# youmi-zym/GO-SLAM

Measured on AMD Instinct MI355X. Metric: BA keyframes/s (6 x FactorGraph.update: reproject + corr lookup + GRU + 2 GN BA iters) on synthetic 640x480 RGB-D, higher is better.
Workload: dtype f32 (BA/geometry; fp64 solve), f16 (corr volume, GRU convs); 1 GPU; configs[1]-shaped frontend window: 60x80 maps (480x640 RGB-D), P=25 keyframes, E=75 edges, 6 updates/keyframe, iters=2, RGB-D depth prior, upsample on; parallelism=replicas x1 (tracking does not shard)

## Files before the change

go_slam_amd/csrc/ba.hip:

```cpp
#include "common.h"

int gs_chol_solve_launch(double* H, double* b, int n, float lm, float ep, float* dx_out, int32_t* fail_flag,
                         int32_t* fail_count, hipStream_t st);

namespace {

constexpr float kMinDepth = 0.25f;
constexpr float kAlpha = 0.05f;
constexpr int kPrepThreads = 1024;
constexpr int kAccSplit = 4;
constexpr int kMaxBuf = 4096;

struct BaWs {
  int32_t* hdr;
  int32_t* kinv;
  int32_t* kx;
  int32_t* edge_m;
  int32_t* row_ptr;
  int32_t* csr_edge;
  int32_t* ent_ptr;
  int32_t* ent_src;
  int32_t* ent_pose;
  int32_t* pair_ptr;
  float* Q;
  float* W;
  float* Ei;
  float* Eij;
  float* part;
  double* H;
  double* b;
  size_t total;
};

BaWs carve(void* base, int E, int P, int M, int nbuf, int hw) {
  BaWs w;
  size_t off = 0;
  auto take = [&](size_t bytes) { size_t o = off; off += gs_align(bytes); return (char*)base + o; };
  w.hdr = (int32_t*)take(16 * 4);
  w.kinv = (int32_t*)take((size_t)nbuf * 4);
  w.kx = (int32_t*)take((size_t)(M + 1) * 4);
  w.edge_m = (int32_t*)take((size_t)(E + 1) * 4);
  w.row_ptr = (int32_t*)take((size_t)(M + 2) * 4);
  w.csr_edge = (int32_t*)take((size_t)(E + 1) * 4);
  w.ent_ptr = (int32_t*)take((size_t)(M + 2) * 4);
  w.ent_src = (int32_t*)take((size_t)(M + E + 1) * 4);
  w.ent_pose = (int32_t*)take((size_t)(M + E + 1) * 4);
  w.pair_ptr = (int32_t*)take((size_t)(M + 2) * 4);
  w.Q = (float*)take((size_t)M * hw * 4);
  w.W = (float*)take((size_t)M * hw * 4);
  w.Ei = (float*)take((size_t)M * 6 * hw * 4);
  w.Eij = (float*)take((size_t)E * 6 * hw * 4);
  w.part = (float*)take((size_t)kAccSplit * M * 8 * hw * 4);
  const size_t n = (size_t)6 * P;
  w.H = (double*)take((n * n + n) * 8);
  w.b = w.H + n * n;
  w.total = off;
  return w;
}

__device__ void block_exclusive_scan(int* data, int n, int* scratch , int* total) {
  const int tid = threadIdx.x;
  const int per = (n + kPrepThreads - 1) / kPrepThreads;
  const int beg = min(tid * per, n), end = min(beg + per, n);
  int s = 0;
  for (int i = beg; i < end; ++i) s += data[i];
  scratch[tid] = s;
  __syncthreads();
  for (int off = 1; off < kPrepThreads; off <<= 1) {
    int v = (tid >= off) ? scratch[tid - off] : 0;
    __syncthreads();
    scratch[tid] += v;
    __syncthreads();
  }
  int run = scratch[tid] - s;
  for (int i = beg; i < end; ++i) {
    int v = data[i];
    data[i] = run;
    run += v;
  }
  if (tid == kPrepThreads - 1) *total = scratch[tid];
  __syncthreads();
}

__global__ __launch_bounds__(kPrepThreads) void ba_prep_kernel(
    const int64_t* __restrict__ ii, const int64_t* __restrict__ jj, int E, int nbuf, int t0, int t1,
    int M_host, BaWs w) {
  __shared__ int flag[kMaxBuf];
  __shared__ int cnt_a[kMaxBuf];
  __shared__ int cnt_b[kMaxBuf];
  __shared__ int scratch[kPrepThreads];
  __shared__ int total;
  const int tid = threadIdx.x;

  for (int k = tid; k < nbuf; k += kPrepThreads) flag[k] = (k >= t0 && k < t1) ? 1 : 0;
  __syncthreads();
  for (int e = tid; e < E; e += kPrepThreads) {
    const int i = (int)ii[e];
    if (i >= 0 && i < nbuf) flag[i] = 1;
  }
  __syncthreads();
  for (int k = tid; k < nbuf; k += kPrepThreads) cnt_a[k] = flag[k];
  __syncthreads();
  block_exclusive_scan(flag, nbuf, scratch, &total);
  const int M_dev = total;
  const int M = min(M_dev, M_host);
  for (int k = tid; k < nbuf; k += kPrepThreads) {
    const bool mem = cnt_a[k] != 0;
    const int r = flag[k];
    const int row = (mem && r < M) ? r : -1;
    w.kinv[k] = row;
    if (row >= 0) w.kx[row] = k;
  }
  if (tid == 0) {
    w.hdr[0] = M_dev;
    w.hdr[1] = (M_dev != M_host) ? 1 : 0;
    w.hdr[2] = 0;
    w.hdr[3] = 0;
  }
  __syncthreads();
  for (int m = tid; m < kMaxBuf; m += kPrepThreads) { cnt_a[m] = 0; cnt_b[m] = 0; }
  __syncthreads();
  for (int k = tid; k < nbuf; k += kPrepThreads) {
    const int row = w.kinv[k];
    if (row >= 0 && k >= t0 && k < t1) cnt_b[row] = 1;
  }
  __syncthreads();
  for (int e = tid; e < E; e += kPrepThreads) {
    const int i = (int)ii[e], j = (int)jj[e];
    const int row = (i >= 0 && i < nbuf) ? w.kinv[i] : -1;
    w.edge_m[e] = row;
    if (row >= 0) {
      atomicAdd(&cnt_a[row], 1);
      if (j >= t0 && j < t1) atomicAdd(&cnt_b[row], 1);
    }
  }
  __syncthreads();
  for (int m = tid; m < M_host; m += kPrepThreads) flag[m] = cnt_b[m] * cnt_b[m];
  __syncthreads();
  block_exclusive_scan(cnt_a, M_host, scratch, &total);
  if (tid == 0) w.row_ptr[M_host] = total;
  block_exclusive_scan(cnt_b, M_host, scratch, &total);
  if (tid == 0) w.ent_ptr[M_host] = total;
  block_exclusive_scan(flag, M_host, scratch, &total);
  if (tid == 0) { w.pair_ptr[M_host] = total; w.hdr[4] = total; }
  __syncthreads();
  for (int m = tid; m < M_host; m += kPrepThreads) {
    w.row_ptr[m] = cnt_a[m];
    w.ent_ptr[m] = cnt_b[m];
    w.pair_ptr[m] = flag[m];
  }
  __syncthreads();
  for (int m = tid; m < M; m += kPrepThreads) {
    int rp = cnt_a[m], ep = cnt_b[m];
    const int k = w.kx[m];
    if (k >= t0 && k < t1) { w.ent_src[ep] = m; w.ent_pose[ep] = k - t0; ++ep; }
    for (int e = 0; e < E; ++e) {
      if (w.edge_m[e] == m) {
        w.csr_edge[rp++] = e;
        const int j = (int)jj[e];
        if (j >= t0 && j < t1) { w.ent_src[ep] = M_host + e; w.ent_pose[ep] = j - t0; ++ep; }
      }
    }
  }
}
// ... 172 lines not shown
          if (j_in) gs_atomic_add_f64(&w.b[6 * pj_ + (tid - 84)], s);
        }
      }
      __syncthreads();
    }
  }

  if (!motion_only && active) {
    if (nsplit > 1) {
      float* po = w.part + (((size_t)split * gridDim.y + m) * 8) * hw + p;
      po[0] = Csum;
      po[(size_t)hw] = wsum;
#pragma unroll
      for (int n = 0; n < 6; ++n) po[(size_t)(2 + n) * hw] = Ei[n];
      return;
    }
    const size_t o = (size_t)m * hw + p;
    const float sens = disps_sens[(size_t)k * hw + p];
    const float mk = (sens > 0.0f) ? 1.0f : 0.0f;
    const float C = Csum + mk * kAlpha + (1.0f - mk) * eta[o];
    const float ww = wsum - mk * kAlpha * (disp - sens);
    w.Q[o] = 1.0f / C;
    w.W[o] = ww;
    if (i_in) {
      float* eo = w.Ei + ((size_t)m * 6) * hw + p;
#pragma unroll
      for (int n = 0; n < 6; ++n) eo[(size_t)n * hw] = Ei[n];
    }
  }
}

__global__ __launch_bounds__(256) void ba_accum_finish_kernel(const float* __restrict__ disps,
                                                              const float* __restrict__ disps_sens,
                                                              const float* __restrict__ eta, int t0, int t1, int hw, int nsp,
                                                              BaWs w) {
  const int m = blockIdx.y;
  if (m >= w.hdr[0]) return;
  const int nsplit = min(nsp, max(w.row_ptr[m + 1] - w.row_ptr[m], 1));
  if (nsplit <= 1) return;
  const int p = blockIdx.x * 256 + threadIdx.x;
  if (p >= hw) return;
  float acc[8];
#pragma unroll
  for (int n = 0; n < 8; ++n) acc[n] = 0.0f;
  for (int s2 = 0; s2 < nsplit; ++s2) {
    const float* pi_ = w.part + (((size_t)s2 * gridDim.y + m) * 8) * hw + p;
#pragma unroll
    for (int n = 0; n < 8; ++n) acc[n] += pi_[(size_t)n * hw];
  }
  const int k = w.kx[m];
  const size_t o = (size_t)m * hw + p;
  const float disp = disps[(size_t)k * hw + p];
  const float sens = disps_sens[(size_t)k * hw + p];
  const float mk = (sens > 0.0f) ? 1.0f : 0.0f;
  const float C = acc[0] + mk * kAlpha + (1.0f - mk) * eta[o];
  const float ww = acc[1] - mk * kAlpha * (disp - sens);
  w.Q[o] = 1.0f / C;
  w.W[o] = ww;
  const int pi = k - t0;
  if (pi >= 0 && pi < t1 - t0) {
    float* eo = w.Ei + ((size_t)m * 6) * hw + p;
#pragma unroll
    for (int n = 0; n < 6; ++n) eo[(size_t)n * hw] = acc[2 + n];
  }
}

__global__ __launch_bounds__(256) void ba_schur_kernel(int M, int hw, int P, BaWs w) {
  __shared__ float red[4][44];
  const int tid = threadIdx.x;
  const int wave = tid >> 6, lane = tid & 63;
  typedef const __attribute__((address_space(4))) int* cip;
  cip pair_ptr = (cip)w.pair_ptr, ent_ptr = (cip)w.ent_ptr, ent_pose = (cip)w.ent_pose, ent_src = (cip)w.ent_src;
  const int n_pairs = pair_ptr[M];
  const int n6 = 6 * P;
  for (int pidx = blockIdx.x; pidx < n_pairs; pidx += gridDim.x) {
    int lo = 0, hi = M;
    while (hi - lo > 1) {
      const int mid = (lo + hi) >> 1;
      if (pair_ptr[mid] <= pidx) lo = mid; else hi = mid;
    }
    const int m = lo;
    const int eb = ent_ptr[m];
    const int nm = ent_ptr[m + 1] - eb;
    const int r = pidx - pair_ptr[m];
    const int a = r / nm, b = r - a * nm;
    const int pa = ent_pose[eb + a], pb = ent_pose[eb + b];
    if (pa < pb) continue;
    const int sa = ent_src[eb + a], sb = ent_src[eb + b];
    const float* Ea = (sa < M) ? w.Ei + (size_t)sa * 6 * hw : w.Eij + (size_t)(sa - M) * 6 * hw;
    const float* Eb = (sb < M) ? w.Ei + (size_t)sb * 6 * hw : w.Eij + (size_t)(sb - M) * 6 * hw;
    const float* Qm = w.Q + (size_t)m * hw;
    const float* Wm = w.W + (size_t)m * hw;
    const bool diag = (a == b);
    float S[36];
#pragma unroll
    for (int i = 0; i < 36; ++i) S[i] = 0.f;
    float vv[6] = {0.f, 0.f, 0.f, 0.f, 0.f, 0.f};
    constexpr int UP = 4;
    for (int p0 = tid; p0 < hw; p0 += UP * 256) {
      float q[UP], ea[UP][6], eb_[UP][6], ww[UP];
#pragma unroll
      for (int u = 0; u < UP; ++u) {
        const int p = p0 + 256 * u;
        const bool ok = p < hw;
        const int pc = ok ? p : tid;
        q[u] = Qm[pc];
#pragma unroll
        for (int n = 0; n < 6; ++n) {
          ea[u][n] = Ea[(size_t)n * hw + pc];
          eb_[u][n] = Eb[(size_t)n * hw + pc];
        }
        ww[u] = diag ? Wm[pc] : 0.0f;
      }
#pragma unroll
      for (int u = 0; u < UP; ++u) {
        if (p0 + 256 * u < hw) {
#pragma unroll
          for (int n = 0; n < 6; ++n) ea[u][n] = ea[u][n] * q[u];
#pragma unroll
          for (int n = 0; n < 6; ++n)
#pragma unroll
            for (int c = 0; c < 6; ++c) S[n * 6 + c] = fmaf(ea[u][n], eb_[u][c], S[n * 6 + c]);
          if (diag) {
#pragma unroll
            for (int n = 0; n < 6; ++n) vv[n] = fmaf(ea[u][n], ww[u], vv[n]);
          }
        }
      }
    }
    {
      float rs[42];
#pragma unroll
      for (int i = 0; i < 36; ++i) rs[i] = S[i];
#pragma unroll
      for (int n = 0; n < 6; ++n) rs[36 + n] = vv[n];
      gs_wave_reduce_scatter<42>(rs, lane);
      const int ix = gs_bitrev6(lane);
      if (ix < 42) red[wave][ix] = rs[0];
    }
    __syncthreads();
    if (tid < 36) {
      const int rr = tid / 6, cc = tid - rr * 6;
      const double s = (double)((red[0][tid] + red[1][tid]) + (red[2][tid] + red[3][tid]));
      if (pa > pb || rr >= cc)
        gs_atomic_add_f64(&w.H[(size_t)(6 * pa + rr) * n6 + (6 * pb + cc)], -s);
    } else if (diag && tid < 42) {
      const double s = (double)((red[0][tid] + red[1][tid]) + (red[2][tid] + red[3][tid]));
      gs_atomic_add_f64(&w.b[6 * pa + (tid - 36)], -s);
    }
    __syncthreads();
  }
}

__global__ __launch_bounds__(256) void ba_update_kernel(
    float* __restrict__ poses, float* __restrict__ disps, const float* __restrict__ dx,
    float* __restrict__ dz, int M, int t0, int t1, int hw, BaWs w) {
  const int tid = threadIdx.x;
  const int P = t1 - t0;
  if ((int)blockIdx.y == M) {
    if (blockIdx.x != 0) return;
    for (int kk = t0 + tid; kk < t1; kk += 256) {
      float* pp = poses + (size_t)kk * 7;
      float t[3] = {pp[0], pp[1], pp[2]};
      float q[4] = {pp[3], pp[4], pp[5], pp[6]};
      float xi[6], tn[3], qn[4];
#pragma unroll
      for (int n = 0; n < 6; ++n) xi[n] = dx[(size_t)(kk - t0) * 6 + n];
      gs_retr_se3(xi, t, q, tn, qn);
      pp[0] = tn[0]; pp[1] = tn[1]; pp[2] = tn[2];
      pp[3] = qn[0]; pp[4] = qn[1]; pp[5] = qn[2]; pp[6] = qn[3];
    }
    return;
  }
  const int m = blockIdx.y;
  const int p = blockIdx.x * 256 + tid;
  if (p >= hw) return;
  if (m >= w.hdr[0]) {
    dz[(size_t)m * hw + p] = 0.0f;
    return;
  }
  const int eb = w.ent_ptr[m], ee = w.ent_ptr[m + 1];
  float dw = 0.f;
  for (int idx = eb; idx < ee; ++idx) {
    const int pn = w.ent_pose[idx];
    if (pn <= 0 || pn >= P) continue;
    const int s = w.ent_src[idx];
    const float* En = (s < M) ? w.Ei + (size_t)s * 6 * hw : w.Eij + (size_t)(s - M) * 6 * hw;
    float acc = 0.f;
#pragma unroll
    for (int n = 0; n < 6; ++n) acc += En[(size_t)n * hw + p] * dx[(size_t)pn * 6 + n];
    dw += acc;
  }
  const size_t o = (size_t)m * hw + p;
  const float z = w.Q[o] * (w.W[o] - dw);
  dz[o] = z;
  const size_t dk = (size_t)w.kx[m] * hw + p;
  disps[dk] = disps[dk] + z;
}

__global__ void ba_status_kernel(int32_t* status_out, BaWs w) {
  if (threadIdx.x < 4) status_out[threadIdx.x] = (threadIdx.x == 2) ? w.hdr[3] : (threadIdx.x == 3 ? w.hdr[4] : w.hdr[threadIdx.x]);
}

}

extern "C" size_t gs_ba_workspace_bytes(int n_edges, int n_poses, int n_depth, int nbuf, int hw) {
  if (n_edges < 0 || n_poses < 0 || n_depth < 0 || nbuf < 0 || hw < 0) return 0;
  return carve(nullptr, n_edges, n_poses, n_depth, nbuf, hw).total + 256;
}

extern "C" int gs_ba_ex(float* poses, float* disps, const float* intrinsics, const float* disps_sens,
                        const float* targets, const float* weights, const float* eta, const int64_t* ii,
                        const int64_t* jj, int t0, int t1, int iterations, float lm, float ep, int motion_only,
                        int n_edges, int n_depth, int nbuf, int h, int w, float* dx, float* dz,
                        int32_t* status_out, void* workspace, size_t workspace_bytes, int flags, gs_stream_t stream) {
  GS_REQUIRE(poses && disps && intrinsics && disps_sens && targets && weights && ii && jj && dx && workspace,
             "ba: null pointer");
  GS_REQUIRE(motion_only || (eta && dz), "ba: eta/dz required unless motion_only");
  GS_REQUIRE(h > 0 && w > 0 && n_edges >= 0 && iterations >= 0, "ba: bad shape");
  GS_REQUIRE(t0 >= 0 && t1 > t0 && t1 <= nbuf, "ba: window [%d,%d) outside buffer of %d frames", t0, t1, nbuf);
  GS_REQUIRE(nbuf <= kMaxBuf, "ba: buffer of %d frames exceeds the supported %d", nbuf, kMaxBuf);
  GS_REQUIRE(n_depth > 0 && n_depth <= nbuf && n_depth <= 65534, "ba: n_depth=%d out of range", n_depth);
  const int hw = h * w, P = t1 - t0, M = n_depth;
  const size_t need = gs_ba_workspace_bytes(n_edges, P, M, nbuf, hw);
  if (workspace_bytes < need) {
    gs_set_error("ba: workspace too small (%zu < %zu bytes)", workspace_bytes, need);
    return GS_ERR_WORKSPACE;
  }
  void* base = (void*)gs_align((size_t)workspace);
  BaWs ws = carve(base, n_edges, P, M, nbuf, hw);
  hipStream_t st = (hipStream_t)stream;
  const int n6 = 6 * P;

  const bool reuse = (flags & 1) != 0;
  if (!reuse) {
    ba_prep_kernel<<<1, kPrepThreads, 0, st>>>(ii, jj, n_edges, nbuf, t0, t1, M, ws);
    GS_CHECK_LAUNCH("ba_prep");
  }
  const int chunks = gs_cdiv(hw, 256);
  for (int it = 0; it < iterations; ++it) {
    if (hipMemsetAsync(ws.H, 0, ((size_t)n6 * n6 + n6) * sizeof(double), st) != hipSuccess) {
      gs_set_error("ba: memset failed");
      return GS_ERR_LAUNCH;
    }
    const int nsp = (!motion_only && n_edges >= 6 * M) ? kAccSplit : 1;
    ba_accum_kernel<<<dim3(chunks, M, nsp), 256, 0, st>>>(poses, disps, intrinsics, disps_sens, targets, weights,
                                                          eta, jj, t0, t1, hw, w, motion_only,
                                                          (reuse && it == 0) ? 1 : 0, ws);
    GS_CHECK_LAUNCH("ba_accum");
    if (!motion_only) {
      if (nsp > 1) {
        ba_accum_finish_kernel<<<dim3(chunks, M), 256, 0, st>>>(disps, disps_sens, eta, t0, t1, hw, nsp, ws);
        GS_CHECK_LAUNCH("ba_accum_finish");
      }
      ba_schur_kernel<<<2048, 256, 0, st>>>(M, hw, P, ws);
      GS_CHECK_LAUNCH("ba_schur");
    }
    int rc = gs_chol_solve_launch(ws.H, ws.b, n6, lm, ep, dx, &ws.hdr[2], &ws.hdr[3], st);
    if (rc != GS_OK) return rc;
    if (motion_only)
      ba_update_kernel<<<dim3(1, 1), 256, 0, st>>>(poses, disps, dx, dz, 0, t0, t1, hw, ws);
    else
      ba_update_kernel<<<dim3(chunks, M + 1), 256, 0, st>>>(poses, disps, dx, dz, M, t0, t1, hw, ws);
    GS_CHECK_LAUNCH("ba_update");
  }
  if (status_out) {
    ba_status_kernel<<<1, 64, 0, st>>>(status_out, ws);
    GS_CHECK_LAUNCH("ba_status");
  }
  return GS_OK;
}

extern "C" int gs_ba(float* poses, float* disps, const float* intrinsics, const float* disps_sens,
                     const float* targets, const float* weights, const float* eta, const int64_t* ii,
                     const int64_t* jj, int t0, int t1, int iterations, float lm, float ep, int motion_only,
                     int n_edges, int n_depth, int nbuf, int h, int w, float* dx, float* dz,
                     int32_t* status_out, void* workspace, size_t workspace_bytes, gs_stream_t stream) {
  return gs_ba_ex(poses, disps, intrinsics, disps_sens, targets, weights, eta, ii, jj, t0, t1, iterations, lm, ep,
                  motion_only, n_edges, n_depth, nbuf, h, w, dx, dz, status_out, workspace, workspace_bytes, 0, stream);
}
```

go_slam_amd/depth_video.py:

```python
import torch
import torch.multiprocessing as _mp

from . import droid_backends
from .droid_net import cvx_upsample


class DepthVideo:
    def __init__(self, cfg_or_ht, args_or_wd, buffer=512, device="cuda:0", stereo=False, full_res=False):
        if isinstance(cfg_or_ht, int):
            self.cfg, self.args = None, None
            mh, mw = int(cfg_or_ht), int(args_or_wd)
            shared = False
        else:
            cfg, args = cfg_or_ht, args_or_wd
            self.cfg, self.args = cfg, args
            mh, mw = cfg["cam"]["H_out"] // 8, cfg["cam"]["W_out"] // 8
            buffer, device = cfg["tracking"]["buffer"], args.device
            stereo = (cfg["mode"] == "stereo")
            full_res, shared = True, True
        self.device = torch.device(device)
        self.scale_factor = 8
        self.map_ht, self.map_wd = mh, mw
        self.ht, self.wd = (cfg["cam"]["H_out"], cfg["cam"]["W_out"]) if self.cfg is not None else (8 * mh, 8 * mw)
        self.stereo = stereo
# ... 81 lines not shown
            self.disps[index] = self.disps_sens[index].clone()
        for slot, name in ((5, "intrinsics"), (6, "fmaps"), (7, "nets"), (8, "inps")):
            if len(item) > slot and (slot > 5 or item[slot] is not None):
                getattr(self, name)[index] = item[slot]
        if len(item) > 6:
            self._run_write_hooks(index)
        if len(item) > 9 and item[9] is not None and hasattr(self, "poses_gt"):
            self.poses_gt[index] = item[9].to(self.poses_gt.device)

    def add_write_hook(self, fn):
        import weakref
        hooks = self.__dict__.setdefault("_write_hooks", [])
        hooks.append(weakref.WeakMethod(fn) if hasattr(fn, "__self__") else (lambda f=fn: f))

    def __getstate__(self):
        state = dict(self.__dict__)
        state.pop("_write_hooks", None)
        return state

    def _run_write_hooks(self, index):
        hooks = self.__dict__.get("_write_hooks")
        if hooks:
            live = []
            for h in hooks:
                fn = h()
                if fn is not None:
                    fn(index)
                    live.append(h)
            self._write_hooks = live

    def __getitem__(self, index):
        if isinstance(index, int) and index > 0:
            index = self._count() + index
        return (self.poses[index], self.disps[index], self.intrinsics[index], self.fmaps[index], self.nets[index],
                self.inps[index])

    def append(self, *item):
        self[self._count()] = item

    def get_bound(self):
        with self.mapping.get_lock():
            return self.bound[0]

    def get_mapping_item(self, index, device="cuda:0", decay=0.1):
        from .lietorch_shim import SE3
        with self.mapping.get_lock():
            image = self.images[index].permute(1, 2, 0).contiguous().to(device)
            mask = self.mask_filtered[index].clone().to(device)
            depth = 1.0 / (self.disps_filtered[index].to(device) + 1e-7)
            w2c = SE3(self.poses_filtered[index].clone()).to(device)
            c2w = (SE3(self.pose_compensate[0].clone()).to(device) * w2c.inv()).matrix()
            gt_c2w = self.poses_gt[index].clone().to(device)
            self.update_priority[index] *= decay
            self._finish_locked_section()
        return image, depth, c2w, gt_c2w, mask

    def get_mapping_items(self, indices, device="cuda:0", decay=0.1):
        from .lietorch_shim import SE3
        order = list(indices)
        uniq = list(dict.fromkeys(order))
        if not uniq:
            return {}
        t = torch.as_tensor(uniq, dtype=torch.long, device=self.images.device)
        count = {}
        for i in order:
            count[i] = count.get(i, 0) + 1
        with self.mapping.get_lock():
            images = self.images[t].permute(0, 2, 3, 1).contiguous().to(device)
            masks = self.mask_filtered[t].clone().to(device)
            depths = 1.0 / (self.disps_filtered[t].to(device) + 1e-7)
            w2c = SE3(self.poses_filtered[t].clone()).to(device)
            c2w = (SE3(self.pose_compensate[0:1].clone()).to(device) * w2c.inv()).matrix()
            gt = self.poses_gt[t].clone().to(device)
            for k in range(max(count.values())):
                sel = [i for i in uniq if count[i] > k]
                self.update_priority[torch.as_tensor(sel, dtype=torch.long, device=self.update_priority.device)] *= decay
            self._finish_locked_section()
        return {i: (images[j], depths[j], c2w[j], gt[j], masks[j]) for j, i in enumerate(uniq)}

    def normalize(self):
        with self.get_lock():
            n = self._count()
            s = self.disps[:n].mean()
            self.disps[:n] /= s
            self.poses[:n, :3] *= s
            self.dirty[:n] = True
            self._finish_locked_section()

    def _finish_locked_section(self):
        if self._shared and self.device.type == "cuda":
            torch.cuda.current_stream(self.device).synchronize()

    @staticmethod
    def format_indices(ii, jj, device="cuda"):
        if not isinstance(ii, torch.Tensor):
            ii = torch.as_tensor(ii)
        if not isinstance(jj, torch.Tensor):
            jj = torch.as_tensor(jj)
        return (ii.to(device=device, dtype=torch.long).reshape(-1).contiguous(),
                jj.to(device=device, dtype=torch.long).reshape(-1).contiguous())

    def upsample(self, ix, mask):
        if hasattr(mask, "upsample_into"):
            ix = ix.to(device=self.device, dtype=torch.long).contiguous()
            if self.disps.is_cuda and self.disps.is_contiguous() and self.disps_up.is_contiguous():
                mask.upsample_into(self.disps, ix, self.disps_up)
                return
            mask = mask.materialize()
        m = mask.reshape(-1, 576, self.map_ht, self.map_wd)
        if m.dtype == torch.float16 and m.is_cuda:
            cl = m.is_contiguous(memory_format=torch.channels_last)
            if not cl:
                m = m.contiguous()
            ix = ix.to(device=self.device, dtype=torch.long).contiguous()
            from . import _lib
            with torch.cuda.device(self.device):
                rc = _lib.lib().gs_cvx_upsample(_lib.ptr(self.disps), _lib.ptr(m), _lib.ptr(ix),
                                                _lib.ptr(self.disps_up), ix.numel(), self.map_ht, self.map_wd, int(cl),
                                                _lib.stream_ptr(self.device))
            _lib.check(rc, "DepthVideo.upsample")
            return
        up = cvx_upsample(self.disps[ix].unsqueeze(-1), mask)
        self.disps_up[ix] = up.squeeze(-1).float()

    def reproject(self, ii, jj):
        ii, jj = DepthVideo.format_indices(ii, jj, self.device)
        return droid_backends.reproject(self.poses, self.disps, self.intrinsics, ii, jj)

    def distance(self, ii=None, jj=None, beta=0.3, bidirectional=True):
        return_matrix = False
        N = self._count()
        if ii is None:
            return_matrix = True
            ii, jj = torch.meshgrid(torch.arange(N), torch.arange(N), indexing="ij")
        ii, jj = DepthVideo.format_indices(ii, jj, self.device)
        intr = self.intrinsics[0].contiguous()
        if bidirectional:
            poses = self.poses[:N].clone()
            d1 = droid_backends.frame_distance(poses, self.disps, intr, ii, jj, beta)
            d2 = droid_backends.frame_distance(poses, self.disps, intr, jj, ii, beta)
            d = 0.5 * (d1 + d2)
        else:
            d = droid_backends.frame_distance(self.poses, self.disps, intr, ii, jj, beta)
        return d.reshape(N, N) if return_matrix else d

    ba_accepts_tables = True

    def ba(self, target, weight, eta, ii, jj, t0=1, t1=None, iters=2, lm=1e-4, ep=0.1,
           motion_only=False, ba_type=None, tables=None):
        lock = self.get_lock() if ba_type is None else self.get_ba_lock(ba_type)
        with lock:
            if t1 is None:
                t1 = max(int(ii.max()), int(jj.max())) + 1
            out = droid_backends.ba(self.poses, self.disps, self.intrinsics[0].contiguous(), self.disps_sens,
                                    target, weight, eta, ii, jj, t0, t1, iters, lm, ep, motion_only, tables=tables)
            self.disps.clamp_(min=0.001)
            self._finish_locked_section()
        return out
```

go_slam_amd/droid_backends.py:

```python
import os

import torch

from . import _lib

_DT = {torch.float16: 0, torch.float32: 1, torch.float64: 2}

_ws_cache = {}
_ba_status = {}
BA_CHECK = os.environ.get("GOSLAM_BA_CHECK", "0") == "1"


def _chk(name, t, dtype=None):
    if not isinstance(t, torch.Tensor):
        raise RuntimeError(f"{name} must be a tensor")
    if not t.is_cuda:
        raise RuntimeError(f"{name} must be a GPU tensor (go_slam_amd has no CPU path)")
    if not t.is_contiguous():
        raise RuntimeError(f"{name} must be contiguous")
    if dtype is not None and t.dtype != dtype:
        raise RuntimeError(f"{name} must have dtype {dtype}, got {t.dtype}")
    return t


def _workspace(device, nbytes):
    key = (device.index, torch.cuda.current_stream(device).cuda_stream)
    buf = _ws_cache.get(key)
    if buf is None or buf.numel() < nbytes:
        buf = torch.empty(int(nbytes * 1.25) + 1024, dtype=torch.uint8, device=device)
        _ws_cache[key] = buf
    return buf


def ba(poses, disps, intrinsics, disps_sens, targets, weights, eta, ii, jj,
       t0, t1, iterations, lm, ep, motion_only, tables=None):
    _chk("targets", targets, torch.float32)
    _chk("weights", weights, torch.float32)
    _chk("poses", poses, torch.float32)
    _chk("disps", disps, torch.float32)
    _chk("intrinsics", intrinsics, torch.float32)
    _chk("disps_sens", disps_sens, torch.float32)
    _chk("ii", ii, torch.int64)
    _chk("jj", jj, torch.int64)
    if not eta.is_contiguous():
        eta = eta.contiguous()
    dev = poses.device
    nbuf, ht, wd = disps.shape
    E = ii.shape[0]
    P = int(t1) - int(t0)
    hw = ht * wd
    M = eta.reshape(-1, hw).shape[0]
    L = _lib.lib()
    need = L.gs_ba_workspace_bytes(E, P, M, nbuf, hw)
    flags = 0
    new_key = None
    if tables is None:
        ws = _workspace(dev, need + 256)
    else:
        key = (ii.data_ptr(), ii._version, jj.data_ptr(), jj._version, E, int(t0), int(t1), M, nbuf, ht, wd, dev)
        ws = tables.get("workspace")
        if ws is not None and tables.get("key") == key and ws.numel() >= need + 256:
            flags = 1
        else:
            ws = tables["workspace"] = torch.empty(need + 256, dtype=torch.uint8, device=dev)
            tables.pop("key", None)
            new_key = key
    dx = torch.empty(P, 6, dtype=torch.float32, device=dev)
    dz = None if motion_only else (torch.empty if int(iterations) > 0 else torch.zeros)(M, hw, dtype=torch.float32,
                                                                                      device=dev)
    status = _ba_status.get(dev.index)
    if status is None:
        status = _ba_status[dev.index] = torch.zeros(4, dtype=torch.int32, device=dev)
    with torch.cuda.device(dev):
        rc = L.gs_ba_ex(_lib.ptr(poses), _lib.ptr(disps), _lib.ptr(intrinsics), _lib.ptr(disps_sens),
                        _lib.ptr(targets), _lib.ptr(weights), _lib.ptr(eta), _lib.ptr(ii), _lib.ptr(jj),
                        int(t0), int(t1), int(iterations), float(lm), float(ep), int(bool(motion_only)),
                        E, M, nbuf, ht, wd, _lib.ptr(dx), _lib.ptr(dz), _lib.ptr(status),
                        _lib.ptr(ws), ws.numel(), flags, _lib.stream_ptr(dev))
    _lib.check(rc, "droid_backends.ba")
    if new_key is not None:
        tables["key"] = new_key
        tables["ii"], tables["jj"] = ii, jj
    if BA_CHECK:
        st = ba_status(dev)
        if st["depth_rows_mismatch"]:
            raise RuntimeError(f"droid_backends.ba: eta has {M} rows but the graph has {st['depth_keyframes']} depth "
                               "keyframes (unique(arange(t0, t1) U ii))")
    return [dx, dz]


def ba_status(device=None):
    dev = torch.device("cuda", torch.cuda.current_device()) if device is None else torch.device(device)
    status = _ba_status.get(dev.index if dev.index is not None else torch.cuda.current_device())
    if status is None:
        return None
    s = status.tolist()
    return {"depth_keyframes": s[0], "depth_rows_mismatch": bool(s[1]), "cholesky_failures": s[2]}


def frame_distance(poses, disps, intrinsics, ii, jj, beta):
    _chk("poses", poses, torch.float32)
    _chk("disps", disps, torch.float32)
    _chk("intrinsics", intrinsics, torch.float32)
    _chk("ii", ii, torch.int64)
    _chk("jj", jj, torch.int64)
    n = ii.shape[0]
    _, ht, wd = disps.shape
    dist = torch.empty(n, dtype=torch.float32, device=poses.device)
    with torch.cuda.device(poses.device):
        rc = _lib.lib().gs_frame_distance(_lib.ptr(poses), _lib.ptr(disps), _lib.ptr(intrinsics), _lib.ptr(ii),
                                          _lib.ptr(jj), _lib.ptr(dist), n, ht, wd, float(beta),
                                          _lib.stream_ptr(poses.device))
    _lib.check(rc, "droid_backends.frame_distance")
    return dist


def projmap(poses, disps, intrinsics, ii, jj):
    _chk("poses", poses, torch.float32)
    _chk("disps", disps, torch.float32)
    _chk("intrinsics", intrinsics, torch.float32)
    _chk("ii", ii, torch.int64)
    _chk("jj", jj, torch.int64)
    n = ii.shape[0]
    _, ht, wd = disps.shape
    coords = torch.empty(n, ht, wd, 3, dtype=torch.float32, device=poses.device)
    valid = torch.empty(n, ht, wd, 1, dtype=torch.float32, device=poses.device)
    with torch.cuda.device(poses.device):
        rc = _lib.lib().gs_projmap(_lib.ptr(poses), _lib.ptr(disps), _lib.ptr(intrinsics), _lib.ptr(ii),
                                   _lib.ptr(jj), _lib.ptr(coords), _lib.ptr(valid), n, ht, wd,
                                   _lib.stream_ptr(poses.device))
    _lib.check(rc, "droid_backends.projmap")
    return [coords, valid]


def depth_filter(poses, disps, intrinsics, ix, thresh):
    _chk("poses", poses, torch.float32)
    _chk("disps", disps, torch.float32)
    _chk("intrinsics", intrinsics, torch.float32)
    _chk("ix", ix, torch.int64)
    _chk("thresh", thresh, torch.float32)
    num, ht, wd = disps.shape
    n = ix.shape[0]
    counter = torch.empty(n, ht, wd, dtype=torch.float32, device=disps.device)
    with torch.cuda.device(disps.device):
        rc = _lib.lib().gs_depth_filter(_lib.ptr(poses), _lib.ptr(disps), _lib.ptr(intrinsics), _lib.ptr(ix),
                                        _lib.ptr(thresh), _lib.ptr(counter), n, num, ht, wd,
                                        _lib.stream_ptr(disps.device))
    _lib.check(rc, "droid_backends.depth_filter")
    return counter


def iproj(poses, disps, intrinsics):
    _chk("poses", poses, torch.float32)
    _chk("disps", disps, torch.float32)
    _chk("intrinsics", intrinsics, torch.float32)
    n, ht, wd = disps.shape
    points = torch.empty(n, ht, wd, 3, dtype=torch.float32, device=disps.device)
    with torch.cuda.device(disps.device):
        rc = _lib.lib().gs_iproj(_lib.ptr(poses), _lib.ptr(disps), _lib.ptr(intrinsics), _lib.ptr(points),
                                 n, ht, wd, _lib.stream_ptr(disps.device))
    _lib.check(rc, "droid_backends.iproj")
    return points


def corr_index_forward(volume, coords, radius):
    _chk("volume", volume)
    _chk("coords", coords, torch.float32)
    if volume.dtype not in _DT:
        raise RuntimeError(f"corr_index_forward: unsupported dtype {volume.dtype}")
    n, h1, w1, h2, w2 = volume.shape
    rd = 2 * radius + 1
    corr = torch.empty(n, rd, rd, h1, w1, dtype=volume.dtype, device=volume.device)
    with torch.cuda.device(volume.device):
        rc = _lib.lib().gs_corr_index_forward(_lib.ptr(volume), _lib.ptr(coords), _lib.ptr(corr), n, h1, w1, h2,
                                              w2, int(radius), _DT[volume.dtype],
                                              _lib.stream_ptr(volume.device))
    _lib.check(rc, "droid_backends.corr_index_forward")
    return [corr]


def corr_index_backward(volume, coords, corr_grad, radius):
    _chk("volume", volume)
    _chk("coords", coords, torch.float32)
    _chk("corr_grad", corr_grad, volume.dtype)
    n, h1, w1, h2, w2 = volume.shape
    grad = torch.zeros_like(volume)
    with torch.cuda.device(volume.device):
        rc = _lib.lib().gs_corr_index_backward(_lib.ptr(coords), _lib.ptr(corr_grad), _lib.ptr(grad), n, h1, w1,
                                               h2, w2, int(radius), _DT[volume.dtype],
                                               _lib.stream_ptr(volume.device))
    _lib.check(rc, "droid_backends.corr_index_backward")
    return [grad]


CORR_ROWMAJOR, CORR_TILE8 = 0, 1


def corr_lookup_pyramid(pyramid, coords, radius=3, channels_last=False, layout=CORR_ROWMAJOR, map_size=None):
    assert len(pyramid) == 4
    for i, v in enumerate(pyramid):
        _chk(f"pyramid[{i}]", v, pyramid[0].dtype)
    _chk("coords", coords, torch.float32)
    if layout == CORR_TILE8:
        n, h1, w1 = pyramid[0].shape[:3]
        h2, w2 = map_size
        for l in range(4):
            want = (n, h1, w1, _lib.lib().gs_corr_level_elems(h2, w2, l, layout)) if l < 2 else (n, h1, w1, h2 >> l, w2 >> l)
            if tuple(pyramid[l].shape) != want:
                raise RuntimeError(f"tile8 pyramid level {l} has shape {tuple(pyramid[l].shape)}, expected {want}")
    else:
        n, h1, w1, h2, w2 = pyramid[0].shape
        for l in range(4):
            if tuple(pyramid[l].shape) != (n, h1, w1, h2 >> l, w2 >> l):
                raise RuntimeError(f"pyramid level {l} has shape {tuple(pyramid[l].shape)}")
    rd = 2 * radius + 1
    corr = torch.empty((n, 4 * rd * rd, h1, w1), dtype=pyramid[0].dtype, device=coords.device,
                       memory_format=torch.channels_last if channels_last else torch.contiguous_format)
    with torch.cuda.device(coords.device):
        rc = _lib.lib().gs_corr_lookup_pyramid(_lib.ptr(pyramid[0]), _lib.ptr(pyramid[1]), _lib.ptr(pyramid[2]),
                                               _lib.ptr(pyramid[3]), _lib.ptr(coords), _lib.ptr(corr), n, h1, w1,
                                               h2, w2, int(radius), _DT[pyramid[0].dtype], int(bool(channels_last)),
                                               int(layout), _lib.stream_ptr(coords.device))
    _lib.check(rc, "corr_lookup_pyramid")
    return corr


def reproject(poses, disps, intrinsics, ii, jj):
    _chk("poses", poses, torch.float32)
    _chk("disps", disps, torch.float32)
    _chk("intrinsics", intrinsics, torch.float32)
    _chk("ii", ii, torch.int64)
    _chk("jj", jj, torch.int64)
    n = ii.shape[0]
    _, ht, wd = disps.shape
    coords = torch.empty(1, n, ht, wd, 2, dtype=torch.float32, device=poses.device)
    valid = torch.empty(1, n, ht, wd, 1, dtype=torch.float32, device=poses.device)
    with torch.cuda.device(poses.device):
        rc = _lib.lib().gs_reproject(_lib.ptr(poses), _lib.ptr(disps), _lib.ptr(intrinsics), _lib.ptr(ii),
                                     _lib.ptr(jj), _lib.ptr(coords), _lib.ptr(valid), n, ht, wd,
                                     _lib.stream_ptr(poses.device))
    _lib.check(rc, "reproject")
# ... 82 lines not shown
```

include/goslam_hip.h:

```cpp
#ifndef GOSLAM_HIP_H
#define GOSLAM_HIP_H

#include <stddef.h>
#include <stdint.h>

#ifdef __cplusplus
extern "C" {
#endif

typedef void* gs_stream_t;

typedef enum {
  GS_OK = 0,
  GS_ERR_INVALID_ARG = -1,
  GS_ERR_WORKSPACE = -2,
  GS_ERR_LAUNCH = -3,
  GS_ERR_UNSUPPORTED = -4
} gs_status;

typedef enum { GS_F16 = 0, GS_F32 = 1, GS_F64 = 2 } gs_dtype;

const char* gs_version(void);
const char* gs_last_error(void);

// ... 29 lines not shown

size_t gs_corr_volume_workspace_bytes(int n, int dim, int h, int w);
size_t gs_corr_level_elems(int h, int w, int level, int layout);
int gs_corr_volume_pyramid(const void* fmap1, const void* fmap2, void* vol0, void* vol1, void* vol2,
                           void* vol3, int n, int dim, int h, int w, int layout,
                           void* workspace, size_t workspace_bytes, gs_stream_t stream);
int gs_corr_volume_pyramid_slots(const void* fmap1, const void* fmap2, void* vol0, void* vol1, void* vol2,
                                 void* vol3, const int64_t* out_slot, int n, int dim, int h, int w, int layout,
                                 void* workspace, size_t workspace_bytes, gs_stream_t stream);

int gs_altcorr_forward(const void* fmap1, const void* fmap2, const float* coords, void* corr,
                       int b, int s, int h1, int w1, int h2, int w2, int c, int radius, int dtype,
                       gs_stream_t stream);

int gs_altcorr_backward(const float* fmap1, const float* fmap2, const float* coords, const float* corr_grad,
                        float* fmap1_grad, float* fmap2_grad, int b, int s, int h1, int w1, int h2, int w2,
                        int c, int radius, gs_stream_t stream);

int gs_altcorr_pyramid(const void* pyr0, const void* pyr1, const void* pyr2, const void* pyr3, const float* coords,
                       const int64_t* ii, const int64_t* jj, void* out, int e, int h, int w, int c, int radius,
                       gs_stream_t stream);


int gs_reproject(const float* poses, const float* disps, const float* intrinsics,
                 const int64_t* ii, const int64_t* jj, float* coords, float* valid,
                 int n, int h, int w, gs_stream_t stream);

int gs_projmap(const float* poses, const float* disps, const float* intrinsics,
               const int64_t* ii, const int64_t* jj, float* coords, float* valid,
               int n, int h, int w, gs_stream_t stream);

int gs_frame_distance(const float* poses, const float* disps, const float* intrinsics,
                      const int64_t* ii, const int64_t* jj, float* dist,
                      int n, int h, int w, float beta, gs_stream_t stream);

int gs_iproj(const float* poses, const float* disps, const float* intrinsics, float* points,
             int n, int h, int w, gs_stream_t stream);

int gs_depth_filter(const float* poses, const float* disps, const float* intrinsics,
                    const int64_t* ix, const float* thresh, float* counter,
                    int n, int num, int h, int w, gs_stream_t stream);

size_t gs_pointcloud_workspace_bytes(int k, int h, int w);
int gs_pointcloud_count(const float* poses, const float* disps, const float* intrinsics, const int64_t* index,
                        const float* disp_floor, float thresh, float visible_num, int k, int num, int h, int w,
                        void* workspace, size_t workspace_bytes, gs_stream_t stream);
int gs_pointcloud_mask(const float* mask, const int64_t* index, int k, int num, int h, int w, void* workspace,
                       size_t workspace_bytes, gs_stream_t stream);
int gs_pointcloud_scan(int k, int h, int w, void* workspace, size_t workspace_bytes, long long* offsets,
                       gs_stream_t stream);
int gs_pointcloud_emit(const float* poses_inv, const float* disps, const float* intrinsics, const float* images,
                       const int64_t* index, int k, int num, int h, int w, const void* workspace,
                       size_t workspace_bytes, long long n_points, float* points, float* colors, gs_stream_t stream);

#define GS_FRAME_PREP_MAX_VIEWS 32
typedef struct {
  const uint8_t* src;
  const float* map_x;
  const float* map_y;
  uint8_t* tmp;
  float* dst;
  int h, w, c, mh, mw;
} gs_color_view;
typedef struct {
  const uint16_t* src;
  float* dst;
  int h, w;
} gs_depth_view;
int gs_frame_prep_color(const gs_color_view* views_host, int n, int H_out, int W_out, int H_edge, int W_edge,
                        gs_stream_t stream);
int gs_frame_prep_depth(const gs_depth_view* views_host, int n, float scale, int H_out, int W_out, int H_edge,
                        int W_edge, gs_stream_t stream);


int gs_gru_gate_zr(const void* zr_pre, const float* bias_zr, const float* glo_zr, const void* inp_pre, void* hx,
                   void* z_out, int n, int hw, int ldx, gs_stream_t stream);
int gs_gru_gate_q(const void* q_pre, const float* bias_q, const float* glo_q, const void* inp_pre, const void* z,
                  const void* net, void* net_out, int n, int hw, gs_stream_t stream);
int gs_bias_act(const void* x, const float* bias, void* y, int rows, int channels, int x_stride, int y_stride,
                int act, gs_stream_t stream);
int gs_motion_features(const float* coords1, const float* target, void* out, int n, int h, int w,
                       gs_stream_t stream);
int gs_lowmem_gather(const float* coords1, const float* target, const void* net, const int64_t* sel,
                     float* coords_out, void* motion_out, void* net_out, int n_sel, int h, int w, gs_stream_t stream);
int gs_lowmem_scatter(const float* coords, const float* delta, const float* weight, const void* net_new,
                      const int64_t* sel, float* target, float* weight_all, void* net, int n_sel, int h, int w,
                      gs_stream_t stream);

int gs_ba_inputs(const float* coords1, const float* delta, const float* weight, float* target,
                 float* ba_target, float* ba_weight, int n, int h, int w, gs_stream_t stream);
int gs_conv1x1(const void* x, int x_stride, int k_in, const void* wpack, const float* bias, int act, void* y,
               int y_stride, int n_out, long long rows, gs_stream_t stream);
int gs_conv7x7_c4(const void* x, const void* wpack, const float* bias, void* y, int ys, int n, int h, int w, int relu,
                  int rt, gs_stream_t stream);
size_t gs_conv3x3_wpack_elems(int c_in, int n_out);
int gs_conv3x3_pp(const void* x, int x_stride, int c_in, const void* wpack, int tw, void* y, int y_stride, int n_out,
                  int n, int h, int w, int xcd_order, gs_stream_t stream);
int gs_conv3x3_bias_relu(const void* x, int x_stride, int c_in, const void* wpack, const float* bias, void* y,
                         int y_stride, int n_out, int n, int h, int w, gs_stream_t stream);
int gs_conv3x3_gru_zr2(const void* net, const void* x_rest, int x_rest_stride, int c_rest, const void* wpack,
                       const float* bias_zr, const float* glo_zr, const void* inp_pre, void* z_out, void* rnet_out,
                       int n, int h, int w, gs_stream_t stream);
int gs_conv3x3_gru_zr(const void* hx, int hx_stride, int c_in, const void* wpack, const float* bias_zr,
                      const float* glo_zr, const void* inp_pre, void* z_out, void* rnet_out, int n, int h, int w,
                      gs_stream_t stream);
int gs_conv3x3_gru_q(const void* rnet, const void* x_rest, int x_rest_stride, int c_rest, const void* wpack,
                     const float* bias_q, const float* glo_q, const void* inp_pre, const void* z, const void* net,
                     void* net_out, int n, int h, int w, gs_stream_t stream);
int gs_conv3x3_head(const void* x, int x_stride, const float* in_bias, int in_relu, const void* wpack,
                    const float* bias, int n_out, int epilogue, float out_scale, float* out, int n, int h, int w,
                    gs_stream_t stream);
int gs_segment_mean(const void* x, int x_stride, const float* in_bias, int in_relu, const int* seg_offsets,
                    const int* seg_edges, void* out, int n_seg, int hw, int channels, gs_stream_t stream);
size_t gs_norm_act_workspace_bytes(int n, int hw, int channels);
size_t gs_norm_act_workspace_bytes_chunks(int n, int chunks, int channels);
size_t gs_enc_conv_wpack_elems(int ksize, int c_in, int c_out);
int gs_enc_conv_stat_chunks(int h_out, int w_out, int c_out);
int gs_enc_conv(const void* x, int x_stride, int c_in, const void* wpack, const void* bias, void* y, int y_stride,
                int c_out, int ksize, int stride, int n, int h, int w, const void* stat_bias, void* stats_ws,
                gs_stream_t stream);
int gs_norm_act(const void* x, const void* bias, const void* skip, void* y, int n, int hw, int channels,
                int instance_norm, int relu_in, int relu_out, float eps, void* workspace, size_t workspace_bytes,
                int stat_chunks, gs_stream_t stream);
size_t gs_gru_glo_workspace_bytes(int n);
int gs_gru_glo(const void* w_pre, const float* w_bias, const void* net, const void* wz, const void* wr,
               const void* wq, const float* bz, const float* br, const float* bq, float* gzr, float* gq,
               int n, int hw, void* workspace, size_t workspace_bytes, gs_stream_t stream);

size_t gs_gru_glo_fused_workspace_bytes(int n, int hw);
int gs_gru_glo_fused(const void* net, int net_stride, const void* w_pack, const float* w_bias, const void* wz,
                     const void* wr, const void* wq, const float* bz, const float* br, const float* bq, float* gzr,
                     float* gq, int n, int hw, void* workspace, size_t workspace_bytes, gs_stream_t stream);

int gs_damping_rows(const float* eta, const int* inv, const int64_t* index, float* damping_buf, float* out,
                    int n_rows, int hw, float scale, float eps, gs_stream_t stream);

int gs_cvx_upsample(const float* disps, const void* mask, const int64_t* ix, float* out,
                    int m, int h, int w, int mask_channels_last, gs_stream_t stream);
int gs_upmask_upsample(const void* x, int x_stride, const void* weight, const float* bias, const float* disps,
                       const int64_t* ix, float* out, int m, int h, int w, gs_stream_t stream);


size_t gs_ba_workspace_bytes(int n_edges, int n_poses, int n_depth, int nbuf, int hw);

int gs_ba(float* poses, float* disps, const float* intrinsics, const float* disps_sens,
          const float* targets, const float* weights, const float* eta,
          const int64_t* ii, const int64_t* jj,
          int t0, int t1, int iterations, float lm, float ep, int motion_only,
          int n_edges, int n_depth, int nbuf, int h, int w,
          float* dx, float* dz, int32_t* status_out,
          void* workspace, size_t workspace_bytes, gs_stream_t stream);

#define GS_BA_REUSE_TABLES 1
int gs_ba_ex(float* poses, float* disps, const float* intrinsics, const float* disps_sens,
             const float* targets, const float* weights, const float* eta,
             const int64_t* ii, const int64_t* jj,
             int t0, int t1, int iterations, float lm, float ep, int motion_only,
             int n_edges, int n_depth, int nbuf, int h, int w,
             float* dx, float* dz, int32_t* status_out,
             void* workspace, size_t workspace_bytes, int flags, gs_stream_t stream);

int gs_chol_solve(double* H, double* b, int n, float lm, float ep, int path, float* dx, int32_t* status,
                  gs_stream_t stream);

int gs_edge_prep(const float* raw, float* d_work, const long long* ex_i, const long long* ex_j, int n_existing,
                 long long* es, int* count, int cap, int i0, int j0, int t, int rad, int nms, float cut, int stereo,
                 int jmin, gs_stream_t stream);
int gs_edge_greedy(const float* raw, const float* sorted_vals, const long long* order, long long* es, int* count,
                   int cap, int i0, int j0, int t, int nms, float thresh, int max_factors, int loop, gs_stream_t stream);

#ifdef __cplusplus
}
#endif
#endif
```

Before: 82.30 keyframes/s.

## Fuse disparity clamp, H zeroing and status write into BA update kernel

```diff
diff --git a/go_slam_amd/csrc/ba.hip b/go_slam_amd/csrc/ba.hip
--- a/go_slam_amd/csrc/ba.hip
+++ b/go_slam_amd/csrc/ba.hip
@@ -10,6 +10,8 @@
 constexpr int kPrepThreads = 1024;
 constexpr int kAccSplit = 4;
 constexpr int kMaxBuf = 4096;
+constexpr float kDispFloor = 0.001f;
+constexpr int kZeroPerWg = 256 * 8;
 
 struct BaWs {
   int32_t* hdr;
@@ -488,9 +490,12 @@
   }
 }
 
+__device__ __forceinline__ float disp_floor(float v) { return v < kDispFloor ? kDispFloor : v; }
+
 __global__ __launch_bounds__(256) void ba_update_kernel(
     float* __restrict__ poses, float* __restrict__ disps, const float* __restrict__ dx,
-    float* __restrict__ dz, int M, int t0, int t1, int hw, BaWs w) {
+    float* __restrict__ dz, int M, int t0, int t1, int hw, int zrows, int nbuf, int clamp,
+    int32_t* __restrict__ status_out, BaWs w) {
   const int tid = threadIdx.x;
   const int P = t1 - t0;
   if ((int)blockIdx.y == M) {
@@ -506,6 +511,24 @@
       pp[0] = tn[0]; pp[1] = tn[1]; pp[2] = tn[2];
       pp[3] = qn[0]; pp[4] = qn[1]; pp[5] = qn[2]; pp[6] = qn[3];
     }
+    if (status_out && tid < 4) status_out[tid] = (tid == 2) ? w.hdr[3] : (tid == 3 ? w.hdr[4] : w.hdr[tid]);
+    return;
+  }
+  if ((int)blockIdx.y > M) {
+    const int zr = (int)blockIdx.y - M - 1;
+    if (zr < zrows) {
+      const size_t nz = (size_t)(6 * P) * (6 * P) + 6 * P;
+      const size_t step = (size_t)zrows * gridDim.x * 256;
+      for (size_t i = ((size_t)zr * gridDim.x + blockIdx.x) * 256 + tid; i < nz; i += step) w.H[i] = 0.0;
+      return;
+    }
+    const int k = zr - zrows;
+    const int p = blockIdx.x * 256 + tid;
+    if (k >= nbuf || p >= hw) return;
+    const int row = (M > 0) ? w.kinv[k] : -1;
+    if (row >= 0 && row < w.hdr[0]) return;
+    const size_t o = (size_t)k * hw + p;
+    disps[o] = disp_floor(disps[o]);
     return;
   }
   const int m = blockIdx.y;
@@ -531,11 +554,17 @@
   const float z = w.Q[o] * (w.W[o] - dw);
   dz[o] = z;
   const size_t dk = (size_t)w.kx[m] * hw + p;
-  disps[dk] = disps[dk] + z;
+  const float dn = disps[dk] + z;
+  disps[dk] = clamp ? disp_floor(dn) : dn;
 }
 
 __global__ void ba_status_kernel(int32_t* status_out, BaWs w) {
   if (threadIdx.x < 4) status_out[threadIdx.x] = (threadIdx.x == 2) ? w.hdr[3] : (threadIdx.x == 3 ? w.hdr[4] : w.hdr[threadIdx.x]);
+}
+
+__global__ __launch_bounds__(256) void disp_floor_kernel(float* __restrict__ disps, size_t n) {
+  const size_t i = (size_t)blockIdx.x * 256 + threadIdx.x;
+  if (i < n) disps[i] = disp_floor(disps[i]);
 }
 
 }
@@ -569,16 +598,20 @@
   const int n6 = 6 * P;
 
   const bool reuse = (flags & 1) != 0;
+  const bool clamp = (flags & 2) != 0;
+  const size_t nz = (size_t)n6 * n6 + n6;
   if (!reuse) {
     ba_prep_kernel<<<1, kPrepThreads, 0, st>>>(ii, jj, n_edges, nbuf, t0, t1, M, ws);
     GS_CHECK_LAUNCH("ba_prep");
-  }
-  const int chunks = gs_cdiv(hw, 256);
-  for (int it = 0; it < iterations; ++it) {
-    if (hipMemsetAsync(ws.H, 0, ((size_t)n6 * n6 + n6) * sizeof(double), st) != hipSuccess) {
+    if (iterations > 0 && hipMemsetAsync(ws.H, 0, nz * sizeof(double), st) != hipSuccess) {
       gs_set_error("ba: memset failed");
       return GS_ERR_LAUNCH;
     }
+  }
+  const int chunks = gs_cdiv(hw, 256);
+  int zrows = (int)((nz + (size_t)chunks * kZeroPerWg - 1) / ((size_t)chunks * kZeroPerWg));
+  zrows = zrows < 1 ? 1 : (zrows > 64 ? 64 : zrows);
+  for (int it = 0; it < iterations; ++it) {
     const int nsp = (!motion_only && n_edges >= 6 * M) ? kAccSplit : 1;
     ba_accum_kernel<<<dim3(chunks, M, nsp), 256, 0, st>>>(poses, disps, intrinsics, disps_sens, targets, weights,
                                                           eta, jj, t0, t1, hw, w, motion_only,
@@ -594,15 +627,23 @@
     }
     int rc = gs_chol_solve_launch(ws.H, ws.b, n6, lm, ep, dx, &ws.hdr[2], &ws.hdr[3], st);
     if (rc != GS_OK) return rc;
-    if (motion_only)
-      ba_update_kernel<<<dim3(1, 1), 256, 0, st>>>(poses, disps, dx, dz, 0, t0, t1, hw, ws);
-    else
-      ba_update_kernel<<<dim3(chunks, M + 1), 256, 0, st>>>(poses, disps, dx, dz, M, t0, t1, hw, ws);
+    const bool last = it + 1 == iterations;
+    const int Mu = motion_only ? 0 : M;
+    const int rows = Mu + 1 + zrows + ((last && clamp) ? nbuf : 0);
+    ba_update_kernel<<<dim3(chunks, rows), 256, 0, st>>>(poses, disps, dx, dz, Mu, t0, t1, hw, zrows, nbuf,
+                                                         (last && clamp) ? 1 : 0, last ? status_out : nullptr, ws);
     GS_CHECK_LAUNCH("ba_update");
   }
-  if (status_out) {
-    ba_status_kernel<<<1, 64, 0, st>>>(status_out, ws);
-    GS_CHECK_LAUNCH("ba_status");
+  if (iterations <= 0) {
+    if (status_out) {
+      ba_status_kernel<<<1, 64, 0, st>>>(status_out, ws);
+      GS_CHECK_LAUNCH("ba_status");
+    }
+    if (clamp) {
+      const size_t n = (size_t)nbuf * hw;
+      disp_floor_kernel<<<(unsigned)((n + 255) / 256), 256, 0, st>>>(disps, n);
+      GS_CHECK_LAUNCH("ba_disp_floor");
+    }
   }
   return GS_OK;
 }
diff --git a/go_slam_amd/depth_video.py b/go_slam_amd/depth_video.py
--- a/go_slam_amd/depth_video.py
+++ b/go_slam_amd/depth_video.py
@@ -257,8 +257,11 @@
         with lock:
             if t1 is None:
                 t1 = max(int(ii.max()), int(jj.max())) + 1
+            fused = getattr(droid_backends.ba, "floors_disps", False)
             out = droid_backends.ba(self.poses, self.disps, self.intrinsics[0].contiguous(), self.disps_sens,
-                                    target, weight, eta, ii, jj, t0, t1, iters, lm, ep, motion_only, tables=tables)
-            self.disps.clamp_(min=0.001)
+                                    target, weight, eta, ii, jj, t0, t1, iters, lm, ep, motion_only, tables=tables,
+                                    **({"clamp_disps": True} if fused else {}))
+            if not fused:
+                self.disps.clamp_(min=0.001)
             self._finish_locked_section()
         return out
diff --git a/go_slam_amd/droid_backends.py b/go_slam_amd/droid_backends.py
--- a/go_slam_amd/droid_backends.py
+++ b/go_slam_amd/droid_backends.py
@@ -33,7 +33,7 @@
 
 
 def ba(poses, disps, intrinsics, disps_sens, targets, weights, eta, ii, jj,
-       t0, t1, iterations, lm, ep, motion_only, tables=None):
+       t0, t1, iterations, lm, ep, motion_only, tables=None, clamp_disps=False):
     _chk("targets", targets, torch.float32)
     _chk("weights", weights, torch.float32)
     _chk("poses", poses, torch.float32)
@@ -65,6 +65,8 @@
             ws = tables["workspace"] = torch.empty(need + 256, dtype=torch.uint8, device=dev)
             tables.pop("key", None)
             new_key = key
+    if clamp_disps:
+        flags |= 2
     dx = torch.empty(P, 6, dtype=torch.float32, device=dev)
     dz = None if motion_only else (torch.empty if int(iterations) > 0 else torch.zeros)(M, hw, dtype=torch.float32,
                                                                                       device=dev)
@@ -77,6 +79,8 @@
                         int(t0), int(t1), int(iterations), float(lm), float(ep), int(bool(motion_only)),
                         E, M, nbuf, ht, wd, _lib.ptr(dx), _lib.ptr(dz), _lib.ptr(status),
                         _lib.ptr(ws), ws.numel(), flags, _lib.stream_ptr(dev))
+    if rc != 0 and tables is not None:
+        tables.pop("key", None)
     _lib.check(rc, "droid_backends.ba")
     if new_key is not None:
         tables["key"] = new_key
@@ -87,6 +91,9 @@
             raise RuntimeError(f"droid_backends.ba: eta has {M} rows but the graph has {st['depth_keyframes']} depth "
                                "keyframes (unique(arange(t0, t1) U ii))")
     return [dx, dz]
+
+
+ba.floors_disps = True
 
 
 def ba_status(device=None):
diff --git a/include/goslam_hip.h b/include/goslam_hip.h
--- a/include/goslam_hip.h
+++ b/include/goslam_hip.h
@@ -205,6 +205,7 @@
           void* workspace, size_t workspace_bytes, gs_stream_t stream);
 
 #define GS_BA_REUSE_TABLES 1
+#define GS_BA_CLAMP_DISPS 2
 int gs_ba_ex(float* poses, float* disps, const float* intrinsics, const float* disps_sens,
              const float* targets, const float* weights, const float* eta,
              const int64_t* ii, const int64_t* jj,
```

Result: no change. 82.72 keyframes/s, median of 6 (+0.5%).
